# CAMMA-public/SelfPose3d

Measured on AMD Instinct MI355X. Metric: multi-view samples/sec (5-view Panoptic, 80x80x20 voxel), higher is better.
Workload: dtype f32

## Files before the change

### __graft_entry__.py

```python
import os
import sys

ROOT = os.path.dirname(os.path.abspath(__file__))
if ROOT not in sys.path:
    sys.path.insert(0, ROOT)


def build() -> None:
    from selfpose3d_amd import build as b
    lib = b.build(force=True, verbose=True)
    assert os.path.exists(lib)
    from oracle import oracle
    oracle.build()
    import selfpose3d_amd
    from selfpose3d_amd import _lib
    l = _lib.load()
    for sym in _lib.EXPORTS:
        assert hasattr(l, sym), sym
    print("build ok:", lib)


def smoke() -> None:
    import numpy as np
    import torch
# ... 29 lines not shown
                                   torch.ones(B, dtype=torch.uint8, device=dev), B, J, hm[1], hm[0], zc, syn.SPACE_SIZE, img, 28)
    torch.cuda.synchronize()
    ref_z, _ = oracle.unproject_fwd([h.numpy() for h in hms], cam, centers, np.ones(B, np.uint8), syn.SPACE_SIZE, zc, img,
                                    want_grids=False)
    want = np.fft.rfft(ref_z.astype(np.float64), n=28, axis=4).transpose(0, 1, 4, 2, 3)
    got = spec.cpu().numpy().reshape(B, J, 15, 4, 4, 4, 4).transpose(0, 1, 2, 3, 5, 4, 6).reshape(B, J, 15, 16, 16)
    dz = float(np.abs(got - want).max())
    assert dz <= 1e-4 * max(1.0, float(np.abs(want).max())), dz
    one = _lib.unproject_one_fwd_zspectrum([h.to(dev)[:, 2:3] for h in hms], _lib.LAYOUT_PLANAR, J, torch.from_numpy(cam).to(dev),
                                           torch.from_numpy(centers).to(dev), torch.ones(B, dtype=torch.uint8, device=dev), B, hm[1],
                                           hm[0], zc, syn.SPACE_SIZE, img, 28)
    torch.cuda.synchronize()
    got1 = one.cpu().numpy().reshape(B, 1, 15, 4, 4, 4, 4).transpose(0, 1, 2, 3, 5, 4, 6).reshape(B, 1, 15, 16, 16)
    d1 = float(np.abs(got1 - want[:, 2:3]).max())
    assert d1 <= 1e-4 * max(1.0, float(np.abs(want[:, 2:3]).max())), d1
    print(f"smoke ok: unprojection max|d|={dc:.2e}, grids exact, NMS indices exact, fused z-spectrum max|d|={dz:.2e}, "
          f"one-channel z-spectrum max|d|={d1:.2e}")


if __name__ == "__main__":
    build()
    if "--smoke" in sys.argv:
        smoke()
```

### include/sp3d.h

```cpp
#ifndef SP3D_H
#define SP3D_H

#include <stdint.h>

#ifdef __cplusplus
extern "C" {
#endif

#define SP3D_ABI_VERSION 3
#define SP3D_MAX_VIEWS 16
#define SP3D_MAX_TOPK 32

#define SP3D_CAM_STRIDE 64
#define SP3D_CAM_R 0
#define SP3D_CAM_T 9
#define SP3D_CAM_F 12
#define SP3D_CAM_C 14
#define SP3D_CAM_K 16
#define SP3D_CAM_P 19
#define SP3D_CAM_A 21
#define SP3D_CAM_W0 27
#define SP3D_CAM_H0 28
#define SP3D_CAM_FLIP 29
#define SP3D_CAM_RXY 32
// ... 164 lines not shown
int sp3d_wino_output(const float *M, float *y, const float *shift, const float *residual, int mode, int B, int X, int Y,
                     int Z, int O, void *stream);
int sp3d_wino_fused(const float *x, const float *U, float *y, const float *shift, const float *residual, int mode, int B,
                    int X, int Y, int Z, int C, int O, void *stream);

int sp3d_wino_fused_split(const float *x, const void *U3, float *y, const float *shift, const float *residual, int mode, int B,
                          int X, int Y, int Z, int C, int O, void *stream);

#define SP3D_CONV3_WINO_YZ 0x100
int sp3d_wino_fused_split64(const float *x, const void *U3, float *y, const float *shift, const float *residual, int mode,
                            int B, int X, int Y, int Z, int C, int O, void *stream);

int sp3d_conv3_split(const float *x, const void *W3, float *y, const float *shift, const float *residual, int mode, int B,
                     int X, int Y, int Z, int C, int O, void *stream);


int sp3d_conv3_split_skip(const float *x, const void *W3, float *y, const float *shift, const float *xs, const void *WS,
                          int B, int X, int Y, int Z, int C, int O, int CS, void *stream);

int sp3d_wino_fused_split64_skip(const float *x, const void *U3, float *y, const float *shift, const float *xs, const void *WS,
                                 int B, int X, int Y, int Z, int C, int O, int CS, void *stream);

int sp3d_upsample2x_scatter(const float *G, float *out, const float *shift, const float *skip, int64_t batch, int X, int Y,
                            int Z, int O, void *stream);

int sp3d_upsample2x_scatter_head(const float *G, float *head, const float *shift, const float *skip, const float *wout,
                                 const float *bout, int64_t batch, int X, int Y, int Z, int O, int J, void *stream);

int sp3d_upconv2x_fused(const float *x, const void *w_split, const float *shift, const float *skip, const float *w_out,
                        const float *b_out, float *out, int64_t batch, int X, int Y, int Z, int CIN, int O, int J, void *stream);
// ... 22 lines not shown
```

### selfpose3d_amd/_lib.py

```python
from __future__ import annotations

import ctypes as C
import os
from typing import Optional, Sequence

import torch

_HERE = os.path.dirname(os.path.abspath(__file__))
_DEFAULT_LIB_PATH = os.path.join(_HERE, "libsp3d.so")
NOPK_LIB_PATH = os.path.join(_HERE, "libsp3d_nopk.so")
LIB_PATH = os.environ.get("SP3D_LIB_PATH") or _DEFAULT_LIB_PATH

LAYOUT_PLANAR = 0
LAYOUT_NHWC = 1
OUT_CHANNELS_LAST = 0x100
HM_BF16 = 0x200
OUT_BF16 = 0x400
HM_ONE_CHANNEL = 0x800
HM_WIDE_MASK = 0x1000
OUT_ZSPECTRUM = 0x2000
HM_ONE_ZSPECTRUM = 0x4000
SCATTER_AUTO, SCATTER_PER_TAP, SCATTER_MERGE = 0, 2, 3
SCATTER_WIDE = 0x100
CONV3_WINO_YZ = 0x100
MAX_VIEWS = 16
MAX_TOPK = 32
ABI_VERSION = 3

_CTYPES = {"p": C.c_void_p, "i": C.c_int, "l": C.c_int64, "f": C.c_float, "d": C.c_double, "s": C.c_char_p}

SIGNATURES = {
    "sp3d_abi_version": "i:",
    "sp3d_camera_finish": "i: p i",
    "sp3d_error_string": "s: i",
    "sp3d_pack_heatmaps": "i: pp iiiiii p",
    "sp3d_pack_heatmaps_ex": "i: pp iiiiiiii p",
    "sp3d_unproject_fwd": "i: p ii ppppp iiiiiiii p ii p",
    "sp3d_unproject_fwd_indexed": "i: p ii pppppp iiiiiiii p ii p",
    "sp3d_unproject_fwd_strided": "i: p ii pppppp iiiiiiii p ii p",
# ... 408 lines not shown
    if int(x.shape[0]) == 0:
        return x.new_zeros((0, int(x.shape[1]), 3))
    return _SoftArgmaxGridFn.apply(x, centers, grid_size, cube_size, beta)


def fetch_ring(ring: torch.Tensor, dst: torch.Tensor, counter: torch.Tensor):
    lib = load()
    assert ring.is_pinned() and ring.dtype == torch.float32 and dst.is_cuda and counter.is_cuda
    R = int(ring.shape[0])
    n = ring[0].numel()
    assert dst.numel() == n and dst.is_contiguous() and ring.is_contiguous()
    check(lib.sp3d_fetch_ring(ring.data_ptr(), dst.data_ptr(), counter.data_ptr(), R, n, _stream(dst.device)),
          "sp3d_fetch_ring")


def maxpool2x(x: torch.Tensor) -> torch.Tensor:
    lib = load()
    B, Cc, X, Y, Z = (int(v) for v in x.shape)
    y = _empty_cl3d(B, Cc, X // 2, Y // 2, Z // 2, x.device)
    check(lib.sp3d_maxpool2x_cl(x.data_ptr(), y.data_ptr(), B, X, Y, Z, Cc, _stream(x.device)), "sp3d_maxpool2x_cl")
    return y


def rfft3d(x: torch.Tensor) -> torch.Tensor:
    lib = load()
    _require_cuda(x, "x")
    if not x.is_contiguous() or x.dtype != torch.float32 or x.dim() < 3:
        raise Sp3dError("rfft3d: x must be a dense fp32 tensor with >= 3 dims")
    SX, SY, SZ = (int(v) for v in x.shape[-3:])
    batch = int(x.numel() // (SX * SY * SZ))
    out = torch.empty(tuple(x.shape[:-1]) + (SZ // 2 + 1,), dtype=torch.complex64, device=x.device)
    check(lib.sp3d_rfft3d(x.data_ptr(), out.data_ptr(), batch, SX, SY, SZ, _stream(x.device)), "sp3d_rfft3d")
    return out
# ... 395 lines not shown


def skip_fold_enabled() -> bool:
    return env_switch("SP3D_FOLD_SKIP", True)


def _require_skip(xs: torch.Tensor, skip_w: torch.Tensor, x: torch.Tensor, CS: int, numel: int, who: str):
    _require_cl3d_f32(xs, who)
    if xs.device != x.device or tuple(xs.shape) != (x.shape[0], CS) + tuple(x.shape[2:]):
        raise Sp3dError(f"{who}: xs must be ({x.shape[0]}, {CS}, ...) on the grid and device of x, got {tuple(xs.shape)} on {xs.device}")
    if skip_w.device != x.device or skip_w.dtype != torch.bfloat16 or not skip_w.is_contiguous() or skip_w.numel() != numel:
        raise Sp3dError(f"{who}: skip_w must be the split records of the ({x.shape[1]}, {CS}, 1, 1, 1) weight on {x.device}; got "
                        f"{tuple(skip_w.shape)}, {skip_w.dtype}, {skip_w.device}, contiguous={skip_w.is_contiguous()}")


def conv3_split_(x: torch.Tensor, W3: torch.Tensor, shift: torch.Tensor, mode: int,
                 residual: Optional[torch.Tensor] = None, *, xs: Optional[torch.Tensor] = None,
                 skip_w: Optional[torch.Tensor] = None, out: Optional[torch.Tensor] = None) -> torch.Tensor:
    lib = load()
    _require_cuda(x, "x")
    B, Cc, X, Y, Z = (int(v) for v in x.shape)
    _require_cl3d_f32(x, "conv3_split_")
    O = int(W3.shape[3])
    dev = x.device
    y = _result_cl3d(out, B, O, X, Y, Z, x, "conv3_split_")
    if xs is not None or skip_w is not None:
        if xs is None or skip_w is None or int(mode) != 1 or residual is not None:
            raise Sp3dError("conv3_split_: the folded skip takes xs AND skip_w, mode 1 and no residual")
        CS = 16
        _require_skip(xs, skip_w, x, CS, CS * O * 6, "conv3_split_")
        check(lib.sp3d_conv3_split_skip(x.data_ptr(), W3.data_ptr(), y.data_ptr(), shift.data_ptr(), xs.data_ptr(),
                                        skip_w.data_ptr(), B, X, Y, Z, Cc, O, CS, _stream(dev)), "sp3d_conv3_split_skip")
        return y
    if residual is not None:
        residual = _as_cl3d(residual)
    check(lib.sp3d_conv3_split(x.data_ptr(), W3.data_ptr(), y.data_ptr(), shift.data_ptr(), _opt(residual), int(mode),
                               B, X, Y, Z, Cc, O, _stream(dev)), "sp3d_conv3_split")
    return y


def quarter_direct_enabled() -> bool:
    return env_switch("SP3D_QUARTER_DIRECT", True)


def quarter_direct_covers(B: int, C: int, O: int, X: int, Y: int, Z: int) -> bool:
    blocks = B * (X // 5) * (Y // 5) * (Z // 5)
    return O == 128 and C in (64, 128) and X % 5 == 0 and Y % 5 == 0 and Z % 5 == 0 and blocks <= 64

# ... 26 lines not shown
    if residual is not None:
        residual = _as_cl3d(residual)
    y = _result_cl3d(out, B, O, X, Y, Z, x, "wino_conv3d_")
    T = B * ((X + 1) // 2) * ((Y + 1) // 2) * ((Z + 1) // 2)
    V = torch.empty((64, T, Cc), dtype=torch.float32, device=x.device)
    check(lib.sp3d_wino_input(x.data_ptr(), V.data_ptr(), B, X, Y, Z, Cc, _stream(x.device)), "sp3d_wino_input")
    M = torch.bmm(V, U)
    check(lib.sp3d_wino_output(M.data_ptr(), y.data_ptr(), shift.data_ptr(), _opt(residual), int(mode), B, X, Y, Z, O,
                               _stream(x.device)), "sp3d_wino_output")
    return y


def wino_fused_conv3d_(x: torch.Tensor, U: torch.Tensor, shift: torch.Tensor, mode: int,
                       residual: Optional[torch.Tensor] = None, U3: Optional[torch.Tensor] = None, *,
                       xs: Optional[torch.Tensor] = None, skip_w: Optional[torch.Tensor] = None,
                       U3yz: Optional[torch.Tensor] = None, out: Optional[torch.Tensor] = None) -> torch.Tensor:
    lib = load()
    _require_cuda(x, "x")
    B, Cc, X, Y, Z = (int(v) for v in x.shape)
    _require_cl3d_f32(x, "wino_fused_conv3d_")
    O = int(U.shape[2])
    y = _result_cl3d(out, B, O, X, Y, Z, x, "wino_fused_conv3d_")
    yz = 0
    if U3yz is not None and U3 is not None and O == 64 and wino_yz_enabled():
        if U3yz.device != x.device or U3yz.dtype != torch.bfloat16 or not U3yz.is_contiguous() or U3yz.numel() != 48 * Cc * O * 3:
            raise Sp3dError(f"wino_fused_conv3d_: U3yz must be wino_yz_weights_split of the ({O}, {Cc}, 3, 3, 3) weight on {x.device}; "
                            f"got {tuple(U3yz.shape)}, {U3yz.dtype}, {U3yz.device}, contiguous={U3yz.is_contiguous()}")
        U3, yz = U3yz, CONV3_WINO_YZ
    if xs is not None or skip_w is not None:
        if xs is None or skip_w is None or U3 is None or int(mode) != 1 or residual is not None:
            raise Sp3dError("wino_fused_conv3d_: the folded skip takes U3, xs AND skip_w, mode 1 and no residual")
        CS = 32
        _require_skip(xs, skip_w, x, CS, CS * O * 3, "wino_fused_conv3d_")
        check(lib.sp3d_wino_fused_split64_skip(x.data_ptr(), U3.data_ptr(), y.data_ptr(), shift.data_ptr(), xs.data_ptr(),
                                               skip_w.data_ptr(), B, X, Y, Z, Cc, O, CS | yz, _stream(x.device)),
              "sp3d_wino_fused_split64_skip")
        return y
    if residual is not None:
        residual = _as_cl3d(residual)
    if U3 is None:
        name, weights = "sp3d_wino_fused", U
    else:
        name, weights = ("sp3d_wino_fused_split64" if O == 64 else "sp3d_wino_fused_split"), U3
    check(getattr(lib, name)(x.data_ptr(), weights.data_ptr(), y.data_ptr(), shift.data_ptr(), _opt(residual), int(mode) | yz,
                             B, X, Y, Z, Cc, O, _stream(x.device)), name)
    return y


def upconv_weights_split(w_gemm: torch.Tensor) -> torch.Tensor:
    Cc, O = int(w_gemm.shape[0]), int(w_gemm.shape[1]) // 8
    U = w_gemm.float().reshape(Cc, 8 * O // 32, 32).permute(1, 0, 2).contiguous()
    pc = wino_weights_split(U, 8)
# ... 91 lines not shown
```

### selfpose3d_amd/csrc/sp3d_conv3_direct.hip

```cpp
#include <hip/hip_runtime.h>
#include <stdint.h>

#include "../../include/sp3d.h"
#include "sp3d_conv3_host.h"
#include "sp3d_split.h"

namespace sp3d {

constexpr int CD_BX = 16, CD_BY = 8, CD_BZ = 4;
constexpr int CD_RX = CD_BX + 2, CD_RY = CD_BY + 2, CD_RZ = CD_BZ + 2, CD_VOX = 8, CD_ROW = CD_RX * CD_VOX, CD_ZP = CD_RY * CD_ROW + 4;
constexpr int CD_PLANE = CD_RZ * CD_ZP;
constexpr int CD_BUF = 2 * CD_PLANE;
constexpr int CD_NV4 = CD_RX * CD_RY * CD_RZ * 2;
constexpr int CD_PROD = 4;
constexpr int CD_PER = (CD_NV4 + 64 * CD_PROD - 1) / (64 * CD_PROD);
constexpr int CD_BUFS = ((CD_BUF / 4 + 63) / 64) * 256;
#ifndef SP3D_WG_ABLATE
#define SP3D_WG_ABLATE 0
#endif
struct CdRec { u32x4 hl, hh, mm; };


#ifdef SP3D_CD_TIMELINE
__device__ unsigned long long *g_cd_tl = nullptr;
#define CD_STAMP(slot) do { __builtin_amdgcn_sched_barrier(0); if (g_cd_tl && blockIdx.x == 0 && lane == 0 && item < 64) { g_cd_tl[(wave * 64 + item) * 4 + (slot)] = __builtin_readcyclecounter(); \
     \
    if (wave == 0 && (slot) == 0 && item == 0) { g_cd_tl[(7 * 64 + 62) * 4 + 0] = wall_clock64(); g_cd_tl[(7 * 64 + 62) * 4 + 1] = __builtin_readcyclecounter(); } \
    if (wave == 0 && (slot) == 3) { g_cd_tl[(7 * 64 + 63) * 4 + 0] = wall_clock64(); g_cd_tl[(7 * 64 + 63) * 4 + 1] = __builtin_readcyclecounter(); } } __builtin_amdgcn_sched_barrier(0); } while (0)
#else
#define CD_STAMP(slot) do { (void)item; } while (0)
#endif

template <int C, int MODE, bool SKIP = false>
__global__ __launch_bounds__(64 * (4 + CD_PROD)) __attribute__((amdgpu_waves_per_eu(2, 2)))
void conv3_split_kernel(const float *__restrict__ x, const unsigned *__restrict__ W3, float *__restrict__ y,
                        const float *__restrict__ shift, const float *__restrict__ res, int B, int X, int Y, int Z, int NBX,
                        int NBY, int NBZ, int nblocks, const float *__restrict__ xs = nullptr,
                        const unsigned *__restrict__ WS = nullptr)
{
    constexpr int O = 32, NCH = C / 8, CS = 16;
    extern __shared__ __attribute__((aligned(16))) unsigned cd_lds[];
    const int tid = threadIdx.x, lane = tid & 63, wave = tid >> 6, t = lane & 31, h = lane >> 5;
    const int my_blocks = ((int)blockIdx.x < nblocks) ? (nblocks - 1 - (int)blockIdx.x) / (int)gridDim.x + 1 : 0;
    const int n_items = my_blocks * NCH;
    auto decode = [&](int item, int &b, int &ox0, int &oy0, int &oz0) {
        int bid = (int)blockIdx.x + (item / NCH) * (int)gridDim.x;
        const int bz = bid % NBZ; bid /= NBZ;
        const int by = bid % NBY; bid /= NBY;
// ... 178 lines not shown
                for (int i = 0; i < 4; ++i) split3(sv[c2][i], lh[i], hm[i]);
#pragma unroll
                for (int i = 0; i < 4; ++i) acc[i] = mfma_bf16(lh[i], ws[c2].hl, acc[i]);
#pragma unroll
                for (int i = 0; i < 4; ++i) acc[i] = mfma_bf16(hm[i], ws[c2].hh, acc[i]);
#pragma unroll
                for (int i = 0; i < 4; ++i) acc[i] = mfma_bf16(hm[i], ws[c2].mm, acc[i]);
            }
        }
        if (cc == NCH - 1) {
            int b, ox0, oy0, oz0;
            decode(item, b, ox0, oy0, oz0);
            if (ox0 + CD_BX <= X && oy0 + CD_BY <= Y && oz0 + CD_BZ <= Z) {
                const float sh = shift[t];
                const int64_t obase = ((((int64_t)b * X + ox0 + 4 * wave) * Y + oy0 + 4 * h) * Z + oz0) * O + t;
#pragma unroll
                for (int i = 0; i < 4; ++i)
#pragma unroll
                    for (int v = 0; v < 16; ++v) {
                        const int64_t idx = obase + (((int64_t)i * Y + (v & 3)) * Z + (v >> 2)) * O;
                        float val = acc[i][v] + sh;
                        if (MODE == 2) val += res[idx];
                        if (MODE >= 1) val = SKIP ? relu_keep_nan(val) : fmaxf(val, 0.0f);
                        if (MODE == 3) val += res[idx];
#if SP3D_W16_ABLATE & 16
                        if (val == 123.456f)
#endif
                        y[idx] = val;
                    }
            } else {
// ... 42 lines not shown


using namespace sp3d;

static int conv3_cu_count(int dev)
{
    static int cu_count[64] = {0};
    if (dev < 0 || dev >= 64) return 256;
    if (cu_count[dev] == 0) {
        int n = 0;
        cu_count[dev] = (hipDeviceGetAttribute(&n, hipDeviceAttributeMultiprocessorCount, dev) == hipSuccess && n > 0) ? n : 256;
    }
    return cu_count[dev];
}

template <int C, int MODE, bool SKIP>
static int conv3_split_launch(const float *x, const void *W3, float *y, const float *shift, const float *residual, const float *xs,
                              const void *WS, int B, int X, int Y, int Z, const Conv3Grid &g, void *stream)
{
    int dev = 0;
    { const hipError_t ed = hipGetDevice(&dev); if (ed != hipSuccess) return (int)ed; }
    const int cus = conv3_cu_count(dev);
    const int rounds = (int)((g.blocks + cus - 1) / cus);
    const int nwg = (int)((g.blocks + rounds - 1) / rounds);
    const size_t lds = (size_t)2 * CD_BUFS * sizeof(unsigned) + 4 * 1024 * sizeof(float);
    static bool attr_dev[64] = {};
    const int slot = (dev < 0 || dev >= 64) ? 63 : dev;
    if (!attr_dev[slot] || slot == 63) {
        const hipError_t ea = hipFuncSetAttribute(reinterpret_cast<const void *>(conv3_split_kernel<C, MODE, SKIP>),
                                                  hipFuncAttributeMaxDynamicSharedMemorySize, (int)lds);
        if (ea != hipSuccess) return (int)ea;
        attr_dev[slot] = true;
    }
    hipLaunchKernelGGL((conv3_split_kernel<C, MODE, SKIP>), dim3((unsigned)nwg), dim3(64 * (4 + CD_PROD)), lds, (hipStream_t)stream, x,
                       reinterpret_cast<const unsigned *>(W3), y, shift, residual, B, X, Y, Z, g.NBX, g.NBY, g.NBZ, (int)g.blocks, xs,
                       reinterpret_cast<const unsigned *>(WS));
    return launch_status();
}

extern "C" int sp3d_conv3_split(const float *x, const void *W3, float *y, const float *shift, const float *residual, int mode,
                                int B, int X, int Y, int Z, int C, int O, void *stream)
{
    if (O == 128) return conv3_split128(x, W3, y, shift, residual, mode, B, X, Y, Z, C, O, stream);
    const Conv3Grid g = conv3_grid(B, X, Y, Z, CD_BX, CD_BY, CD_BZ);
    const bool supported = O == 32 && (C == 16 || C == 32) && !((reinterpret_cast<uintptr_t>(W3) | reinterpret_cast<uintptr_t>(y)) & 15);
    const bool in_range = (int64_t)X * Y * Z * C * 2 <= 0x7fffffff && g.blocks <= 0x7fffffff;
    if (const int rc = conv3_check(B, X, Y, Z, mode, x && W3 && y && shift && (mode < 2 || residual), supported, in_range)) return rc;
    return with_mode(mode, [&](auto m) {
        constexpr int M = decltype(m)::value;
        return C == 16 ? conv3_split_launch<16, M, false>(x, W3, y, shift, residual, nullptr, nullptr, B, X, Y, Z, g, stream)
                       : conv3_split_launch<32, M, false>(x, W3, y, shift, residual, nullptr, nullptr, B, X, Y, Z, g, stream);
    });
}

extern "C" int sp3d_conv3_split_skip(const float *x, const void *W3, float *y, const float *shift, const float *xs,
                                     const void *WS, int B, int X, int Y, int Z, int C, int O, int CS, void *stream)
{
    const Conv3Grid g = conv3_grid(B, X, Y, Z, CD_BX, CD_BY, CD_BZ);
    const bool supported = O == 32 && C == 32 && CS == 16 &&
                           !((reinterpret_cast<uintptr_t>(W3) | reinterpret_cast<uintptr_t>(WS) | reinterpret_cast<uintptr_t>(xs) |
                              reinterpret_cast<uintptr_t>(y)) & 15);
    const bool in_range = (int64_t)X * Y * Z * C * 2 <= 0x7fffffff && g.blocks <= 0x7fffffff;
    if (const int rc = conv3_check(B, X, Y, Z, 1, x && W3 && y && shift && xs && WS, supported, in_range)) return rc;
    return conv3_split_launch<32, 1, true>(x, W3, y, shift, nullptr, xs, WS, B, X, Y, Z, g, stream);
}


extern "C" int sp3d_debug_conv3_timeline(void *dev_buffer)
{
#ifdef SP3D_CD_TIMELINE
    unsigned long long *p = (unsigned long long *)dev_buffer;
    return (int)hipMemcpyToSymbol(HIP_SYMBOL(sp3d::g_cd_tl), &p, sizeof(p));
#else
    (void)dev_buffer;
    return SP3D_EUNSUPPORTED;
#endif
}
```

### selfpose3d_amd/csrc/sp3d_wino_fused.hip

```cpp
#include <hip/hip_runtime.h>
#include <stdint.h>

#include "../../include/sp3d.h"
#include "sp3d_conv3_host.h"
#include "sp3d_split.h"


namespace sp3d {

#ifdef SP3D_WF_TIMELINE
__device__ unsigned long long *g_wf_tl = nullptr;
#define WF_STAMP(slot) do { __builtin_amdgcn_sched_barrier(0); if (tl && lane == 0) tl[slot] = __builtin_readcyclecounter(); __builtin_amdgcn_sched_barrier(0); } while (0)
#else
#define WF_STAMP(slot) do { } while (0)
#endif

constexpr int WF_RX = 10, WF_RY = 10, WF_RZ = 6;
constexpr int WF_VS = 8;
constexpr int WF_ROW = WF_RX * WF_VS + 4;
constexpr int WF_LDS = WF_RY * WF_RZ * WF_ROW;

__device__ constexpr int wf_ta(int r) { return r == 0 ? 0 : (r == 1 ? 1 : (r == 2 ? 2 : 1)); }
__device__ constexpr int wf_tb(int r) { return r == 0 ? 2 : (r == 1 ? 2 : (r == 2 ? 1 : 3)); }
__device__ constexpr float wf_sb(int r) { return r == 1 ? 1.0f : -1.0f; }
// ... 371 lines not shown
            }
        }
    }
}

typedef float f32x4 __attribute__((ext_vector_type(4)));
constexpr int W16_RX = 10, W16_RY = 10, W16_RZ = 4, W16_VS = 16;
constexpr int W16_ROW = W16_RX * W16_VS + 4;
constexpr int W16_LDS = W16_RY * W16_RZ * W16_ROW;

__device__ __forceinline__ f32x4 mfma16_bf16(u32x4 a, u32x4 b, f32x4 c)
{
    return __builtin_amdgcn_mfma_f32_16x16x32_bf16(__builtin_bit_cast(bf16x8, a), __builtin_bit_cast(bf16x8, b), c, 0, 0, 0);
}

template <int C, int MODE, int NBW, int KS, bool SKIP = false, bool XD = false>
__global__ __launch_bounds__(64 * (4 / NBW) * KS) __attribute__((amdgpu_waves_per_eu(NBW <= 2 ? 2 : 1))) void wino_fused16_kernel(const float *__restrict__ x,
                                                                          const unsigned *__restrict__ U3,
                                                                          float *__restrict__ y, const float *__restrict__ shift,
                                                                          const float *__restrict__ res, int B, int X, int Y,
                                                                          int Z, int NBX, int NBY, int NBZ,
                                                                          const float *__restrict__ xs = nullptr,
                                                                          const unsigned *__restrict__ WS = nullptr)
{
    constexpr int O = 64, NCH = C / 16, NOW = 4 / NBW, NTG = 64 * NOW;
    static_assert(NCH % KS == 0, "chunks must divide evenly over the channel groups");
    __shared__ __attribute__((aligned(16))) float lds[KS * W16_LDS];
    const int tid = threadIdx.x, lane = tid & 63, wave = tid >> 6;
    const int kg = wave / NOW, ow = wave % NOW, tg = tid - kg * NTG;
    float *region = lds + kg * W16_LDS;
    const int tl = lane & 15, q = lane >> 4;
// ... 244 lines not shown
        for (int n = 0; n < NBW; ++n) {
            const int o = (ow * NBW + n) * 16 + tl;
            const float sh = shift[o];
            const int64_t obase = ((((int64_t)b * X + ox0) * Y + oy0) * Z + oz0) * O + o;
            int off[4];
#pragma unroll
            for (int v = 0; v < 4; ++v) off[v] = ((2 * v * Y + 2 * q) * Z) * O;
            float rv[8][4];
            if (MODE >= 2) {
#pragma unroll
                for (int a = 0; a < 8; ++a)
#pragma unroll
                    for (int v = 0; v < 4; ++v)
                        rv[a][v] = res[obase + off[v] + (((a >> 2) * Y + ((a >> 1) & 1)) * Z + (a & 1)) * O];
            }
#pragma unroll
            for (int a = 0; a < 8; ++a)
#pragma unroll
                for (int v = 0; v < 4; ++v) {
                    float val = acc[a][n][v] + sh;
                    if (MODE == 2) val += rv[a][v];
                    if (MODE >= 1) val = SKIP ? relu_keep_nan(val) : fmaxf(val, 0.0f);
                    if (MODE == 3) val += rv[a][v];
                    y[obase + off[v] + (((a >> 2) * Y + ((a >> 1) & 1)) * Z + (a & 1)) * O] = val;
                }
        }
        return;
    }
#pragma unroll
    for (int n = 0; n < NBW; ++n) {
        const int o = (ow * NBW + n) * 16 + tl;
        const float sh = shift[o];
        float rv[8][4];
        if (MODE >= 2) {
#pragma unroll
            for (int a = 0; a < 8; ++a)
#pragma unroll
                for (int v = 0; v < 4; ++v) {
                    const int tile = 4 * q + v;
                    const int rx = tile & 3, ry = tile >> 2;
// ... 88 lines not shown
                           (const float *)nullptr, (const unsigned *)nullptr);
    };
    with_mode(mode, [&](auto m) {
        if (yz) { if (C == 32) launch(int_c<32>{}, m, std::true_type{}); else launch(int_c<64>{}, m, std::true_type{}); }
        else { if (C == 32) launch(int_c<32>{}, m, std::false_type{}); else launch(int_c<64>{}, m, std::false_type{}); }
    });
    return launch_status();
}

extern "C" int sp3d_wino_fused_split64_skip(const float *x, const void *U3, float *y, const float *shift, const float *xs,
                                            const void *WS, int B, int X, int Y, int Z, int C, int O, int CS, void *stream)
{
    const Conv3Grid g = conv3_grid(B, X, Y, Z, 8, 8, 2);
    const bool yz = CS >= 0 && (CS & SP3D_CONV3_WINO_YZ);
    if (yz) CS &= ~SP3D_CONV3_WINO_YZ;
    const bool supported = O == 64 && C == 64 && CS == 32 && !((reinterpret_cast<uintptr_t>(U3) | reinterpret_cast<uintptr_t>(WS)) & 7) &&
                           !(reinterpret_cast<uintptr_t>(xs) & 15);
    const bool in_range = (int64_t)X * Y * Z * CS <= 0x7fffffff && g.blocks <= 0x7fffffff;
    if (const int rc = conv3_check(B, X, Y, Z, 1, x && U3 && y && shift && xs && WS, supported, in_range)) return rc;
    auto launch = [&](auto xd) {
        hipLaunchKernelGGL((wino_fused16_kernel<64, 1, W16_NBW, W16_KS, true, decltype(xd)::value>), dim3((unsigned)g.blocks),
                           dim3(64 * (4 / W16_NBW) * W16_KS), 0, (hipStream_t)stream, x, reinterpret_cast<const unsigned *>(U3), y,
                           shift, (const float *)nullptr, B, X, Y, Z, g.NBX, g.NBY, g.NBZ, xs, reinterpret_cast<const unsigned *>(WS));
    };
    if (yz) launch(std::true_type{}); else launch(std::false_type{});
    return launch_status();
}
```

### selfpose3d_amd/v2v_net.py

```python
from __future__ import annotations

from typing import NamedTuple, Optional

import torch
import torch.nn as nn
import torch.nn.functional as F


def _bn(c):
    from .grouped_bn import GroupedBatchNorm3d
    return GroupedBatchNorm3d(c)


def _grouped(bn, training: bool) -> bool:
    return training and getattr(bn, "groups", None) is not None


def fft_len(n: int) -> int:
    m = n + (n & 1)
    while True:
        r, odd = m, 0
        for q in (2, 3, 5, 7, 11, 13):
            if q > 2 and r % q == 0:
                odd += 1
# ... 198 lines not shown
    w: torch.Tensor
    shift: torch.Tensor
    u: Optional[torch.Tensor] = None
    split: Optional[torch.Tensor] = None
    direct: Optional[torch.Tensor] = None
    direct24: Optional[torch.Tensor] = None
    split_yz: Optional[torch.Tensor] = None


class _Res(NamedTuple):
    c1: _Conv
    c2: _Conv
    skip: Optional[torch.Tensor]
    skip_direct: Optional[torch.Tensor] = None
    skip_split: Optional[torch.Tensor] = None


class _Up(NamedTuple):
    wT: torch.Tensor
    shift: torch.Tensor
    wg: torch.Tensor
    split: Optional[torch.Tensor] = None


class _FoldedV2V:

    def __init__(self, net: "V2VNet"):
        self.net = net
        self.key = None
        self.layers = {}
        self.spectra = {}
        self.xpad = {}

    def graph_tensors(self):
        return dict(self.layers), dict(self.spectra), dict(self.xpad)

    @staticmethod
    def _key(net):
        ps = list(net.parameters()) + list(net.buffers())
        w3 = net.front_layers[1].res_branch[0].weight
        return (tuple((p.data_ptr(), p._version) for p in ps), str(w3.device), bool(is_cl(w3)))

    def _ensure_built(self):
        key = self._key(self.net)
        if key != self.key:
            self._build()
            self.key = key
# ... 33 lines not shown
        ed = n.encoder_decoder
        for name in ("front_res", "encoder_res1", "encoder_res2", "mid_res", "decoder_res2", "decoder_res1", "skip_res1",
                     "skip_res2"):
            blk = n.front_layers[1] if name == "front_res" else getattr(ed, name)
            w1, s1 = self._fold(blk.res_branch[0], blk.res_branch[1])
            w2, s2 = self._fold(blk.res_branch[3], blk.res_branch[4])
            ws = sd = sp = None
            if len(blk.skip_con) > 0:
                ws, ss = self._fold(blk.skip_con[0], blk.skip_con[1])
                s2 = (s2 + ss).contiguous()
                co, ci = int(ws.shape[0]), int(ws.shape[1])
                if ws.is_cuda and (co, ci) == (32, 16):
                    sd = _lib.conv_weights_split(ws)
                if ws.is_cuda and (co, ci) == (64, 32):
                    sp = _lib.wino_weights_split(ws.reshape(co, ci).t().reshape(1, ci, co).contiguous(), 16)
            layers[name] = _Res(self._conv3_record(w1, s1), self._conv3_record(w2, s2), ws, sd, sp)
        for name in ("decoder_upsample2", "decoder_upsample1"):
            blk = getattr(ed, name).block
            wT, sT = self._fold(blk[0], blk[1], transposed=True)
            wg = wT.permute(0, 2, 3, 4, 1).reshape(wT.shape[0], 8 * wT.shape[1]).contiguous()
            fused = wg.is_cuda and (int(wT.shape[0]), int(wT.shape[1])) in ((128, 64), (64, 32))
            layers[name] = _Up(wT, sT, wg, _lib.upconv_weights_split(wg) if fused else None)
        self.layers, self.spectra, self.xpad = layers, {}, {}

    def _route(self, x, c: "_Conv") -> str:
        from . import _lib
        n = self.net
        if c.u is None or not is_cl(x):
            return "library"
        return conv3_route(int(c.w.shape[1]), int(c.w.shape[0]), (x.shape[0],) + tuple(x.shape[2:]), n.winograd,
                           getattr(n, "wino_split", True), getattr(n, "direct_conv", True),
                           quarter_direct=c.direct24 is not None and _lib.quarter_direct_enabled())

    def _conv3(self, x, c: "_Conv", mode, residual=None, xs=None, skip_w=None):
        from . import _lib
        route = self._route(x, c)
        split = getattr(self.net, "wino_split", True)
        if route == "conv3_split_":
            return _lib.conv3_split_(x, c.direct, c.shift, mode, residual, xs=xs, skip_w=skip_w)
        if route == "wino_fused_conv3d_":
            return _lib.wino_fused_conv3d_(x, c.u, c.shift, mode, residual, c.split if split else None, xs=xs, skip_w=skip_w,
                                           U3yz=c.split_yz if split else None)
        assert xs is None and skip_w is None, route
        if route == "conv3_split128_":
            return _lib.conv3_split128_(x, c.direct24, c.shift, mode, residual)
        if route == "wino_conv3d_":
            return _lib.wino_conv3d_(x, c.u, c.shift, mode, residual)
        return _lib.channel_shift_act_(F.conv3d(x, c.w, None, 1, 1), c.shift, mode, residual)

    def _folded_skip(self, x, h, r: "_Res"):
        from . import _lib
        if r.skip is None or not _lib.skip_fold_enabled() or not (is_cl(x) and x.is_cuda and x.dtype == torch.float32):
            return None
        route, widths = self._route(h, r.c2), (int(r.c2.w.shape[1]), int(r.c2.w.shape[0]), int(x.shape[1]))
        if route == "conv3_split_" and widths == (32, 32, 16):
            return r.skip_direct
        if route == "wino_fused_conv3d_" and getattr(self.net, "wino_split", True) and widths == (64, 64, 32):
            return r.skip_split
        return None

    def _res(self, x, name):
        r = self.layers[name]
        h = self._conv3(x, r.c1, 1)
        if r.skip is None:
            return self._conv3(h, r.c2, 2, x)
        rec = self._folded_skip(x, h, r)
        if rec is not None:
            return self._conv3(h, r.c2, 1, xs=x, skip_w=rec)
        return self._conv3(h, r.c2, 2, self._conv1(x, r.skip))

    _tuned_shapes: "set[tuple]" = set()
    _tune_gemms = None

    @staticmethod
    def _tunable():
        from . import _lib
        on = _FoldedV2V._tune_gemms
        if on is None:
            on = _lib.env_switch("SP3D_TUNE_GEMM", False)
        return getattr(torch.cuda, "tunable", None) if on else None

    def _run_tuned(self, x):
# ... 157 lines not shown
        x = self._res(self._pool(x), "encoder_res1")
        skip2 = self._res(x, "skip_res2")
        x = self._res(self._pool(x), "encoder_res2")
        x = self._res(self._res(x, "mid_res"), "decoder_res2")
        x = self._up2x(x, "decoder_upsample2", skip2)
        x = self._res(x, "decoder_res1")
        o = self.net.output_layer
        wT, sT, wg, w3 = self.layers["decoder_upsample1"]
        if self.net.winograd and is_cl(x) and wg.is_cuda and wT.shape[1] == 32 and x.dtype == torch.float32:
            return _lib.upsample2x_head_(x, wg, sT, skip1, o.weight, o.bias, w3)
        x = self._up2x(x, "decoder_upsample1", skip1)
        return self._conv1(x, o.weight, o.bias)

    def _pool(self, x):
        from . import _lib
        if is_cl(x) and x.is_cuda and x.dtype == torch.float32 and x.shape[1] % 4 == 0 and \
                all(int(v) % 2 == 0 for v in x.shape[2:]):
            return _lib.maxpool2x(x)
        return F.max_pool3d(x, 2, 2)

    def _up2x(self, x, name, skip):
        from . import _lib
        wT, sT, wg, w3 = self.layers[name]
        if self.net.winograd and is_cl(x) and wg.is_cuda and wT.shape[1] % 4 == 0:
            return _lib.upsample2x_(x, wg, sT, skip, w3)
        return _lib.channel_shift_act_(F.conv_transpose3d(x, wT, None, 2), sT, 3, skip)

    def _conv1(self, x, w, bias=None):
        if self.net.winograd and is_cl(x) and x.is_cuda:
            B, C, X, Y, Z = x.shape
            O = w.shape[0]
            x2 = x.permute(0, 2, 3, 4, 1).reshape(-1, C)
            y = torch.matmul(x2, w.reshape(O, C).t()) if bias is None else torch.addmm(bias, x2, w.reshape(O, C).t())
# ... 112 lines not shown
```

Before: 2917.

## Fuse 2x max-pool into folded-skip residual conv epilogues

Adds a POOL template variant to the direct and Winograd folded-skip conv kernels. Their epilogue now also writes the 2x2x2 max-pooled output into a trailing buffer. The V2V net uses this for front_res and encoder_res1, so the following _pool call reuses the stashed pooled tensor instead of launching a separate maxpool kernel that re-reads the full activation. This costs extra registers and stores in the conv epilogue, and only applies when the dimensions tile evenly.

```diff
diff --git a/__graft_entry__.py b/__graft_entry__.py
--- a/__graft_entry__.py
+++ b/__graft_entry__.py
@@ -67,8 +67,30 @@
     got1 = one.cpu().numpy().reshape(B, 1, 15, 4, 4, 4, 4).transpose(0, 1, 2, 3, 5, 4, 6).reshape(B, 1, 15, 16, 16)
     d1 = float(np.abs(got1 - want[:, 2:3]).max())
     assert d1 <= 1e-4 * max(1.0, float(np.abs(want[:, 2:3]).max())), d1
+    g = torch.Generator().manual_seed(5)
+    cl = torch.channels_last_3d
+    for kind, (Cc, O, CS), (X, Y, Z) in (("direct", (32, 32, 16), (16, 8, 4)), ("wino", (64, 64, 32), (8, 8, 2))):
+        h = torch.randn(1, Cc, X, Y, Z, generator=g).to(dev).contiguous(memory_format=cl)
+        xs = torch.randn(1, CS, X, Y, Z, generator=g).to(dev).contiguous(memory_format=cl)
+        w2 = (torch.randn(O, Cc, 3, 3, 3, generator=g) / (27 * Cc) ** 0.5).to(dev)
+        ws = (torch.randn(O, CS, 1, 1, 1, generator=g) / CS ** 0.5).to(dev)
+        sh = (0.5 * torch.randn(O, generator=g)).to(dev)
+        if kind == "direct":
+            def run(**kw):
+                return _lib.conv3_split_(h, _lib.conv_weights_split(w2), sh, 1, xs=xs, skip_w=_lib.conv_weights_split(ws), **kw)
+        else:
+            U = _lib.wino_weights(w2)
+            S = _lib.wino_weights_split(ws.reshape(O, CS).t().reshape(1, CS, O).contiguous(), 16)
+
+            def run(**kw):
+                return _lib.wino_fused_conv3d_(h, U, sh, 1, None, _lib.wino_weights_split(U, 16), xs=xs, skip_w=S,
+                                               U3yz=_lib.wino_yz_weights_split(w2), **kw)
+        plain = run()
+        y, yp = run(pool=True)
+        torch.cuda.synchronize()
+        assert torch.equal(y, plain) and torch.equal(yp, _lib.maxpool2x(plain)) and float(yp.max()) > 0.0, kind
     print(f"smoke ok: unprojection max|d|={dc:.2e}, grids exact, NMS indices exact, fused z-spectrum max|d|={dz:.2e}, "
-          f"one-channel z-spectrum max|d|={d1:.2e}")
+          f"one-channel z-spectrum max|d|={d1:.2e}, pooled convs exact")
 
 
 if __name__ == "__main__":
diff --git a/include/sp3d.h b/include/sp3d.h
--- a/include/sp3d.h
+++ b/include/sp3d.h
@@ -202,6 +202,7 @@
 int sp3d_conv3_split(const float *x, const void *W3, float *y, const float *shift, const float *residual, int mode, int B,
                      int X, int Y, int Z, int C, int O, void *stream);
 
+#define SP3D_CONV3_POOL2X 0x200
 
 int sp3d_conv3_split_skip(const float *x, const void *W3, float *y, const float *shift, const float *xs, const void *WS,
                           int B, int X, int Y, int Z, int C, int O, int CS, void *stream);
diff --git a/selfpose3d_amd/_lib.py b/selfpose3d_amd/_lib.py
--- a/selfpose3d_amd/_lib.py
+++ b/selfpose3d_amd/_lib.py
@@ -23,6 +23,7 @@
 SCATTER_AUTO, SCATTER_PER_TAP, SCATTER_MERGE = 0, 2, 3
 SCATTER_WIDE = 0x100
 CONV3_WINO_YZ = 0x100
+CONV3_POOL2X = 0x200
 MAX_VIEWS = 16
 MAX_TOPK = 32
 ABI_VERSION = 3
@@ -461,9 +462,15 @@
           "sp3d_fetch_ring")
 
 
-def maxpool2x(x: torch.Tensor) -> torch.Tensor:
-    lib = load()
+def maxpool2x(x: torch.Tensor, have: Optional[torch.Tensor] = None) -> torch.Tensor:
     B, Cc, X, Y, Z = (int(v) for v in x.shape)
+    if have is not None:
+        if tuple(have.shape) != (B, Cc, X // 2, Y // 2, Z // 2) or have.device != x.device or have.dtype != torch.float32 or \
+                x.dtype != torch.float32 or not have.is_contiguous(memory_format=torch.channels_last_3d):
+            raise Sp3dError(f"maxpool2x: have must be the float32 channels_last_3d ({B}, {Cc}, {X // 2}, {Y // 2}, {Z // 2}) pooled "
+                            f"form of x on {x.device}; got {tuple(have.shape)}, {have.dtype}, {have.device}")
+        return have
+    lib = load()
     y = _empty_cl3d(B, Cc, X // 2, Y // 2, Z // 2, x.device)
     check(lib.sp3d_maxpool2x_cl(x.data_ptr(), y.data_ptr(), B, X, Y, Z, Cc, _stream(x.device)), "sp3d_maxpool2x_cl")
     return y
@@ -889,24 +896,58 @@
                         f"{tuple(skip_w.shape)}, {skip_w.dtype}, {skip_w.device}, contiguous={skip_w.is_contiguous()}")
 
 
+POOL_FOLD_DEFAULT = True
+
+
+def pool_fold_enabled() -> bool:
+    return env_switch("SP3D_FOLD_POOL", POOL_FOLD_DEFAULT)
+
+
+def pool_fold_covers(route: str, X: int, Y: int, Z: int) -> bool:
+    X, Y, Z = int(X), int(Y), int(Z)
+    if min(X, Y, Z) <= 0:
+        return False
+    if route == "conv3_split_":
+        return X % 16 == 0 and Y % 8 == 0 and Z % 4 == 0
+    if route == "wino_fused_conv3d_":
+        return X % 8 == 0 and Y % 8 == 0 and Z % 2 == 0
+    return False
+
+
+def _result_pooled(out: Optional[torch.Tensor], B: int, O: int, X: int, Y: int, Z: int, x: torch.Tensor, who: str):
+    n, npool = B * X * Y * Z * O, B * (X // 2) * (Y // 2) * (Z // 2) * O
+    if out is None:
+        out = torch.empty(n + npool, dtype=torch.float32, device=x.device)
+    elif out.dim() != 1 or out.numel() != n + npool or out.dtype != torch.float32 or out.device != x.device or not out.is_contiguous():
+        raise Sp3dError(f"{who}: with pool=True out must be a dense 1-D float32 buffer of {n} + {npool} elements on {x.device}, got "
+                        f"{tuple(out.shape)}, {out.dtype}, {out.device}")
+    return (out[:n].view(B, X, Y, Z, O).permute(0, 4, 1, 2, 3), out[n:].view(B, X // 2, Y // 2, Z // 2, O).permute(0, 4, 1, 2, 3))
+
+
 def conv3_split_(x: torch.Tensor, W3: torch.Tensor, shift: torch.Tensor, mode: int,
                  residual: Optional[torch.Tensor] = None, *, xs: Optional[torch.Tensor] = None,
-                 skip_w: Optional[torch.Tensor] = None, out: Optional[torch.Tensor] = None) -> torch.Tensor:
+                 skip_w: Optional[torch.Tensor] = None, pool: bool = False, out: Optional[torch.Tensor] = None):
     lib = load()
     _require_cuda(x, "x")
     B, Cc, X, Y, Z = (int(v) for v in x.shape)
     _require_cl3d_f32(x, "conv3_split_")
     O = int(W3.shape[3])
     dev = x.device
-    y = _result_cl3d(out, B, O, X, Y, Z, x, "conv3_split_")
+    if pool:
+        if xs is None or skip_w is None:
+            raise Sp3dError("conv3_split_: pool=True is a form of the folded skip (xs and skip_w)")
+        y, yp = _result_pooled(out, B, O, X, Y, Z, x, "conv3_split_")
+    else:
+        y = _result_cl3d(out, B, O, X, Y, Z, x, "conv3_split_")
     if xs is not None or skip_w is not None:
         if xs is None or skip_w is None or int(mode) != 1 or residual is not None:
             raise Sp3dError("conv3_split_: the folded skip takes xs AND skip_w, mode 1 and no residual")
         CS = 16
         _require_skip(xs, skip_w, x, CS, CS * O * 6, "conv3_split_")
         check(lib.sp3d_conv3_split_skip(x.data_ptr(), W3.data_ptr(), y.data_ptr(), shift.data_ptr(), xs.data_ptr(),
-                                        skip_w.data_ptr(), B, X, Y, Z, Cc, O, CS, _stream(dev)), "sp3d_conv3_split_skip")
-        return y
+                                        skip_w.data_ptr(), B, X, Y, Z, Cc, O, CS | (CONV3_POOL2X if pool else 0), _stream(dev)),
+              "sp3d_conv3_split_skip")
+        return (y, yp) if pool else y
     if residual is not None:
         residual = _as_cl3d(residual)
     check(lib.sp3d_conv3_split(x.data_ptr(), W3.data_ptr(), y.data_ptr(), shift.data_ptr(), _opt(residual), int(mode),
@@ -963,13 +1004,18 @@
 def wino_fused_conv3d_(x: torch.Tensor, U: torch.Tensor, shift: torch.Tensor, mode: int,
                        residual: Optional[torch.Tensor] = None, U3: Optional[torch.Tensor] = None, *,
                        xs: Optional[torch.Tensor] = None, skip_w: Optional[torch.Tensor] = None,
-                       U3yz: Optional[torch.Tensor] = None, out: Optional[torch.Tensor] = None) -> torch.Tensor:
+                       U3yz: Optional[torch.Tensor] = None, pool: bool = False, out: Optional[torch.Tensor] = None):
     lib = load()
     _require_cuda(x, "x")
     B, Cc, X, Y, Z = (int(v) for v in x.shape)
     _require_cl3d_f32(x, "wino_fused_conv3d_")
     O = int(U.shape[2])
-    y = _result_cl3d(out, B, O, X, Y, Z, x, "wino_fused_conv3d_")
+    if pool:
+        if xs is None or skip_w is None:
+            raise Sp3dError("wino_fused_conv3d_: pool=True is a form of the folded skip (U3, xs and skip_w)")
+        y, yp = _result_pooled(out, B, O, X, Y, Z, x, "wino_fused_conv3d_")
+    else:
+        y = _result_cl3d(out, B, O, X, Y, Z, x, "wino_fused_conv3d_")
     yz = 0
     if U3yz is not None and U3 is not None and O == 64 and wino_yz_enabled():
         if U3yz.device != x.device or U3yz.dtype != torch.bfloat16 or not U3yz.is_contiguous() or U3yz.numel() != 48 * Cc * O * 3:
@@ -982,9 +1028,10 @@
         CS = 32
         _require_skip(xs, skip_w, x, CS, CS * O * 3, "wino_fused_conv3d_")
         check(lib.sp3d_wino_fused_split64_skip(x.data_ptr(), U3.data_ptr(), y.data_ptr(), shift.data_ptr(), xs.data_ptr(),
-                                               skip_w.data_ptr(), B, X, Y, Z, Cc, O, CS | yz, _stream(x.device)),
+                                               skip_w.data_ptr(), B, X, Y, Z, Cc, O, CS | yz | (CONV3_POOL2X if pool else 0),
+                                               _stream(x.device)),
               "sp3d_wino_fused_split64_skip")
-        return y
+        return (y, yp) if pool else y
     if residual is not None:
         residual = _as_cl3d(residual)
     if U3 is None:
diff --git a/selfpose3d_amd/csrc/sp3d_conv3_direct.hip b/selfpose3d_amd/csrc/sp3d_conv3_direct.hip
--- a/selfpose3d_amd/csrc/sp3d_conv3_direct.hip
+++ b/selfpose3d_amd/csrc/sp3d_conv3_direct.hip
@@ -31,7 +31,7 @@
 #define CD_STAMP(slot) do { (void)item; } while (0)
 #endif
 
-template <int C, int MODE, bool SKIP = false>
+template <int C, int MODE, bool SKIP = false, bool POOL = false>
 __global__ __launch_bounds__(64 * (4 + CD_PROD)) __attribute__((amdgpu_waves_per_eu(2, 2)))
 void conv3_split_kernel(const float *__restrict__ x, const unsigned *__restrict__ W3, float *__restrict__ y,
                         const float *__restrict__ shift, const float *__restrict__ res, int B, int X, int Y, int Z, int NBX,
@@ -240,6 +240,33 @@
             if (ox0 + CD_BX <= X && oy0 + CD_BY <= Y && oz0 + CD_BZ <= Z) {
                 const float sh = shift[t];
                 const int64_t obase = ((((int64_t)b * X + ox0 + 4 * wave) * Y + oy0 + 4 * h) * Z + oz0) * O + t;
+                if (POOL) {
+                    static_assert(!POOL || (SKIP && MODE == 1), "the pooled form exists for the folded skip only");
+#pragma unroll
+                    for (int i = 0; i < 4; ++i)
+#pragma unroll
+                        for (int v = 0; v < 16; ++v) {
+                            acc[i][v] = relu_keep_nan(acc[i][v] + sh);
+                            y[obase + (((int64_t)i * Y + (v & 3)) * Z + (v >> 2)) * O] = acc[i][v];
+                        }
+                    const int XP = X >> 1, YP = Y >> 1, ZP = Z >> 1;
+                    float *yp = y + (int64_t)B * X * Y * Z * O;
+                    const int64_t pbase = ((((int64_t)b * XP + ((ox0 + 4 * wave) >> 1)) * YP + ((oy0 + 4 * h) >> 1)) * ZP + (oz0 >> 1)) * O + t;
+#pragma unroll
+                    for (int ci = 0; ci < 2; ++ci)
+#pragma unroll
+                        for (int cy = 0; cy < 2; ++cy)
+#pragma unroll
+                            for (int cz = 0; cz < 2; ++cz) {
+                                float m = acc[2 * ci][8 * cz + 2 * cy];
+#pragma unroll
+                                for (int s = 1; s < 8; ++s) {
+                                    const float val = acc[2 * ci + (s >> 2)][4 * (2 * cz + (s & 1)) + 2 * cy + ((s >> 1) & 1)];
+                                    m = (val > m || val != val) ? val : m;
+                                }
+                                yp[pbase + (((int64_t)ci * YP + cy) * ZP + cz) * O] = m;
+                            }
+                } else
 #pragma unroll
                 for (int i = 0; i < 4; ++i)
 #pragma unroll
@@ -312,7 +339,7 @@
     return cu_count[dev];
 }
 
-template <int C, int MODE, bool SKIP>
+template <int C, int MODE, bool SKIP, bool POOL = false>
 static int conv3_split_launch(const float *x, const void *W3, float *y, const float *shift, const float *residual, const float *xs,
                               const void *WS, int B, int X, int Y, int Z, const Conv3Grid &g, void *stream)
 {
@@ -325,12 +352,12 @@
     static bool attr_dev[64] = {};
     const int slot = (dev < 0 || dev >= 64) ? 63 : dev;
     if (!attr_dev[slot] || slot == 63) {
-        const hipError_t ea = hipFuncSetAttribute(reinterpret_cast<const void *>(conv3_split_kernel<C, MODE, SKIP>),
+        const hipError_t ea = hipFuncSetAttribute(reinterpret_cast<const void *>(conv3_split_kernel<C, MODE, SKIP, POOL>),
                                                   hipFuncAttributeMaxDynamicSharedMemorySize, (int)lds);
         if (ea != hipSuccess) return (int)ea;
         attr_dev[slot] = true;
     }
-    hipLaunchKernelGGL((conv3_split_kernel<C, MODE, SKIP>), dim3((unsigned)nwg), dim3(64 * (4 + CD_PROD)), lds, (hipStream_t)stream, x,
+    hipLaunchKernelGGL((conv3_split_kernel<C, MODE, SKIP, POOL>), dim3((unsigned)nwg), dim3(64 * (4 + CD_PROD)), lds, (hipStream_t)stream, x,
                        reinterpret_cast<const unsigned *>(W3), y, shift, residual, B, X, Y, Z, g.NBX, g.NBY, g.NBZ, (int)g.blocks, xs,
                        reinterpret_cast<const unsigned *>(WS));
     return launch_status();
@@ -355,11 +382,15 @@
                                      const void *WS, int B, int X, int Y, int Z, int C, int O, int CS, void *stream)
 {
     const Conv3Grid g = conv3_grid(B, X, Y, Z, CD_BX, CD_BY, CD_BZ);
-    const bool supported = O == 32 && C == 32 && CS == 16 &&
+    const bool pool = CS >= 0 && (CS & SP3D_CONV3_POOL2X);
+    if (pool) CS &= ~SP3D_CONV3_POOL2X;
+    const bool whole = X % CD_BX == 0 && Y % CD_BY == 0 && Z % CD_BZ == 0;
+    const bool supported = O == 32 && C == 32 && CS == 16 && (!pool || whole) &&
                            !((reinterpret_cast<uintptr_t>(W3) | reinterpret_cast<uintptr_t>(WS) | reinterpret_cast<uintptr_t>(xs) |
                               reinterpret_cast<uintptr_t>(y)) & 15);
     const bool in_range = (int64_t)X * Y * Z * C * 2 <= 0x7fffffff && g.blocks <= 0x7fffffff;
     if (const int rc = conv3_check(B, X, Y, Z, 1, x && W3 && y && shift && xs && WS, supported, in_range)) return rc;
+    if (pool) return conv3_split_launch<32, 1, true, true>(x, W3, y, shift, nullptr, xs, WS, B, X, Y, Z, g, stream);
     return conv3_split_launch<32, 1, true>(x, W3, y, shift, nullptr, xs, WS, B, X, Y, Z, g, stream);
 }
 
diff --git a/selfpose3d_amd/csrc/sp3d_wino_fused.hip b/selfpose3d_amd/csrc/sp3d_wino_fused.hip
--- a/selfpose3d_amd/csrc/sp3d_wino_fused.hip
+++ b/selfpose3d_amd/csrc/sp3d_wino_fused.hip
@@ -409,7 +409,7 @@
     return __builtin_amdgcn_mfma_f32_16x16x32_bf16(__builtin_bit_cast(bf16x8, a), __builtin_bit_cast(bf16x8, b), c, 0, 0, 0);
 }
 
-template <int C, int MODE, int NBW, int KS, bool SKIP = false, bool XD = false>
+template <int C, int MODE, int NBW, int KS, bool SKIP = false, bool XD = false, bool POOL = false>
 __global__ __launch_bounds__(64 * (4 / NBW) * KS) __attribute__((amdgpu_waves_per_eu(NBW <= 2 ? 2 : 1))) void wino_fused16_kernel(const float *__restrict__ x,
                                                                           const unsigned *__restrict__ U3,
                                                                           float *__restrict__ y, const float *__restrict__ shift,
@@ -684,6 +684,7 @@
                     for (int v = 0; v < 4; ++v)
                         rv[a][v] = res[obase + off[v] + (((a >> 2) * Y + ((a >> 1) & 1)) * Z + (a & 1)) * O];
             }
+            float pm[4] = {0.0f, 0.0f, 0.0f, 0.0f};
 #pragma unroll
             for (int a = 0; a < 8; ++a)
 #pragma unroll
@@ -693,7 +694,16 @@
                     if (MODE >= 1) val = SKIP ? relu_keep_nan(val) : fmaxf(val, 0.0f);
                     if (MODE == 3) val += rv[a][v];
                     y[obase + off[v] + (((a >> 2) * Y + ((a >> 1) & 1)) * Z + (a & 1)) * O] = val;
-                }
+                    if (POOL) pm[v] = (a == 0) ? val : ((val > pm[v] || val != val) ? val : pm[v]);
+                }
+            if (POOL) {
+                static_assert(!POOL || (SKIP && MODE == 1), "the pooled form exists for the folded skip only");
+                const int XP = X >> 1, YP = Y >> 1, ZP = Z >> 1;
+                float *yp = y + (int64_t)B * X * Y * Z * O;
+                const int64_t pbase = ((((int64_t)b * XP + (ox0 >> 1)) * YP + (oy0 >> 1) + q) * ZP + (oz0 >> 1)) * O + o;
+#pragma unroll
+                for (int v = 0; v < 4; ++v) yp[pbase + (int64_t)v * YP * ZP * O] = pm[v];
+            }
         }
         return;
     }
@@ -812,15 +822,21 @@
     const Conv3Grid g = conv3_grid(B, X, Y, Z, 8, 8, 2);
     const bool yz = CS >= 0 && (CS & SP3D_CONV3_WINO_YZ);
     if (yz) CS &= ~SP3D_CONV3_WINO_YZ;
-    const bool supported = O == 64 && C == 64 && CS == 32 && !((reinterpret_cast<uintptr_t>(U3) | reinterpret_cast<uintptr_t>(WS)) & 7) &&
+    const bool pool = CS >= 0 && (CS & SP3D_CONV3_POOL2X);
+    if (pool) CS &= ~SP3D_CONV3_POOL2X;
+    const bool whole = X % 8 == 0 && Y % 8 == 0 && Z % 2 == 0;
+    const bool supported = O == 64 && C == 64 && CS == 32 && (!pool || whole) &&
+                           !((reinterpret_cast<uintptr_t>(U3) | reinterpret_cast<uintptr_t>(WS)) & 7) &&
                            !(reinterpret_cast<uintptr_t>(xs) & 15);
     const bool in_range = (int64_t)X * Y * Z * CS <= 0x7fffffff && g.blocks <= 0x7fffffff;
     if (const int rc = conv3_check(B, X, Y, Z, 1, x && U3 && y && shift && xs && WS, supported, in_range)) return rc;
-    auto launch = [&](auto xd) {
-        hipLaunchKernelGGL((wino_fused16_kernel<64, 1, W16_NBW, W16_KS, true, decltype(xd)::value>), dim3((unsigned)g.blocks),
-                           dim3(64 * (4 / W16_NBW) * W16_KS), 0, (hipStream_t)stream, x, reinterpret_cast<const unsigned *>(U3), y,
-                           shift, (const float *)nullptr, B, X, Y, Z, g.NBX, g.NBY, g.NBZ, xs, reinterpret_cast<const unsigned *>(WS));
+    auto launch = [&](auto xd, auto pl) {
+        hipLaunchKernelGGL((wino_fused16_kernel<64, 1, W16_NBW, W16_KS, true, decltype(xd)::value, decltype(pl)::value>),
+                           dim3((unsigned)g.blocks), dim3(64 * (4 / W16_NBW) * W16_KS), 0, (hipStream_t)stream, x,
+                           reinterpret_cast<const unsigned *>(U3), y, shift, (const float *)nullptr, B, X, Y, Z, g.NBX, g.NBY, g.NBZ, xs,
+                           reinterpret_cast<const unsigned *>(WS));
     };
-    if (yz) launch(std::true_type{}); else launch(std::false_type{});
+    if (pool) { if (yz) launch(std::true_type{}, std::true_type{}); else launch(std::false_type{}, std::true_type{}); }
+    else { if (yz) launch(std::true_type{}, std::false_type{}); else launch(std::false_type{}, std::false_type{}); }
     return launch_status();
 }
diff --git a/selfpose3d_amd/v2v_net.py b/selfpose3d_amd/v2v_net.py
--- a/selfpose3d_amd/v2v_net.py
+++ b/selfpose3d_amd/v2v_net.py
@@ -236,6 +236,7 @@
     skip: Optional[torch.Tensor]
     skip_direct: Optional[torch.Tensor] = None
     skip_split: Optional[torch.Tensor] = None
+    pooled: bool = False
 
 
 class _Up(NamedTuple):
@@ -253,6 +254,7 @@
         self.layers = {}
         self.spectra = {}
         self.xpad = {}
+        self.pooled = None
 
     def graph_tensors(self):
         return dict(self.layers), dict(self.spectra), dict(self.xpad)
@@ -316,7 +318,8 @@
                     sd = _lib.conv_weights_split(ws)
                 if ws.is_cuda and (co, ci) == (64, 32):
                     sp = _lib.wino_weights_split(ws.reshape(co, ci).t().reshape(1, ci, co).contiguous(), 16)
-            layers[name] = _Res(self._conv3_record(w1, s1), self._conv3_record(w2, s2), ws, sd, sp)
+            layers[name] = _Res(self._conv3_record(w1, s1), self._conv3_record(w2, s2), ws, sd, sp,
+                                pooled=name in ("front_res", "encoder_res1"))
         for name in ("decoder_upsample2", "decoder_upsample1"):
             blk = getattr(ed, name).block
             wT, sT = self._fold(blk[0], blk[1], transposed=True)
@@ -334,16 +337,17 @@
                            getattr(n, "wino_split", True), getattr(n, "direct_conv", True),
                            quarter_direct=c.direct24 is not None and _lib.quarter_direct_enabled())
 
-    def _conv3(self, x, c: "_Conv", mode, residual=None, xs=None, skip_w=None):
+    def _conv3(self, x, c: "_Conv", mode, residual=None, xs=None, skip_w=None, pool=False):
         from . import _lib
         route = self._route(x, c)
         split = getattr(self.net, "wino_split", True)
+        kw = dict(pool=True) if pool else {}
         if route == "conv3_split_":
-            return _lib.conv3_split_(x, c.direct, c.shift, mode, residual, xs=xs, skip_w=skip_w)
+            return _lib.conv3_split_(x, c.direct, c.shift, mode, residual, xs=xs, skip_w=skip_w, **kw)
         if route == "wino_fused_conv3d_":
             return _lib.wino_fused_conv3d_(x, c.u, c.shift, mode, residual, c.split if split else None, xs=xs, skip_w=skip_w,
-                                           U3yz=c.split_yz if split else None)
-        assert xs is None and skip_w is None, route
+                                           U3yz=c.split_yz if split else None, **kw)
+        assert xs is None and skip_w is None and not pool, route
         if route == "conv3_split128_":
             return _lib.conv3_split128_(x, c.direct24, c.shift, mode, residual)
         if route == "wino_conv3d_":
@@ -361,6 +365,10 @@
             return r.skip_split
         return None
 
+    def _pool_fold(self, h, c: "_Conv") -> bool:
+        from . import _lib
+        return bool(_lib.pool_fold_enabled() and _lib.pool_fold_covers(self._route(h, c), *h.shape[2:]))
+
     def _res(self, x, name):
         r = self.layers[name]
         h = self._conv3(x, r.c1, 1)
@@ -368,6 +376,10 @@
             return self._conv3(h, r.c2, 2, x)
         rec = self._folded_skip(x, h, r)
         if rec is not None:
+            if r.pooled and self._pool_fold(h, r.c2):
+                y, yp = self._conv3(h, r.c2, 1, xs=x, skip_w=rec, pool=True)
+                self.pooled = (y, yp)
+                return y
             return self._conv3(h, r.c2, 1, xs=x, skip_w=rec)
         return self._conv3(h, r.c2, 2, self._conv1(x, r.skip))
 
@@ -555,9 +567,11 @@
 
     def _pool(self, x):
         from . import _lib
+        stash, self.pooled = self.pooled, None
+        have = stash[1] if stash is not None and stash[0] is x else None
         if is_cl(x) and x.is_cuda and x.dtype == torch.float32 and x.shape[1] % 4 == 0 and \
                 all(int(v) % 2 == 0 for v in x.shape[2:]):
-            return _lib.maxpool2x(x)
+            return _lib.maxpool2x(x, have=have) if have is not None else _lib.maxpool2x(x)
         return F.max_pool3d(x, 2, 2)
 
     def _up2x(self, x, name, skip):
```

Measured after the change: 2958 (median of 6 runs). 1.01x the previous value.
